# rvp-group/mad-icp

Hardware: NVIDIA H100
Metric: scans/sec (130k-pt scan vs 16-keyframe model) (higher is better)
Workload: dtype f64

## Files before the change

### include/madicp_b200_debug.h

```cpp
#ifndef MADICP_B200_DEBUG_H
#define MADICP_B200_DEBUG_H

#include "madicp_b200.h"

#ifdef __cplusplus
extern "C" {
#endif

int madicp_debug_timing(madicp_ctx_t* ctx, int enable, int64_t* out, int max_rounds);
int madicp_debug_cta_cycles(madicp_ctx_t* ctx, int64_t* out, int cap);
int madicp_debug_cta_stamps(madicp_ctx_t* ctx, int plane, int64_t* out, int cap);
int madicp_set_gn_grid(madicp_ctx_t* ctx, int threads_per_cta, int ctas_per_sm);


int madicp_debug_set_memo(madicp_ctx_t* ctx, int mode);

int64_t madicp_debug_sort_check(int64_t n, uint32_t seed, int64_t distinct, int num_threads);

int64_t madicp_debug_range_mask(const madicp_points_t* desc, uint8_t* keep);

int64_t madicp_debug_correct_points(const madicp_points_t* desc, const madicp_vcorr_t* vcorr, double* out);

int madicp_debug_deskew_plan(const madicp_points_t* desc, const madicp_vcorr_t* vcorr, const double T_prev[12],
                             const double T_now[12], double sensor_hz, int split, int num_threads, int32_t* perm,
                             uint16_t* chunk, double* poses, int* n_poses, int64_t* n_kept);

#ifdef __cplusplus
}
#endif
#endif
```

### mad_icp_b200/_capi.py

```python
import ctypes as C
import os

import numpy as np

_HERE = os.path.dirname(os.path.abspath(__file__))
LIB_PATH = os.path.join(_HERE, "lib", "libmadicp_b200.so")
_lib = None

dp = C.POINTER(C.c_double)
ip = C.POINTER(C.c_int32)
bp = C.POINTER(C.c_uint8)
vp = C.c_void_p


class Points(C.Structure):
    _fields_ = [("data", C.c_void_p), ("n", C.c_int64), ("stride", C.c_int64), ("offset", C.c_int32 * 3),
                ("is_f32", C.c_int32), ("min_range", C.c_double), ("max_range", C.c_double), ("range_mode", C.c_int32),
                ("drop_nan", C.c_int32)]


assert C.sizeof(Points) == 64
pts_p = C.POINTER(Points)


# ... 35 lines not shown
    "madicp_stage_discard": (C.c_int, [vp]),
    "madtree_gpu_upload": (C.c_int, [vp, vp, C.POINTER(vp)]),
    "madtree_gpu_free": (None, [vp]),
    "madtree_gpu_num_nodes": (C.c_int, [vp]),
    "madtree_gpu_num_leaves": (C.c_int, [vp]),
    "madtree_gpu_num_levels": (C.c_int, [vp]),
    "madtree_gpu_download": (C.c_int, [vp, vp, ip]),
    "madtree_gpu_export": (C.c_int, [vp, dp, dp, dp, ip]),
    "madicp_set_moving_tree": (C.c_int, [vp, vp]),
    "madicp_get_moving": (C.c_int, [vp, dp, C.c_int]),
    "madicp_ingest": (C.c_int, [vp, vp, C.c_int64, C.c_int, C.c_int, dp, dp, C.c_double, C.c_int, dp]),
    "madicp_ingest_points": (C.c_int, [vp, pts_p, C.c_int, dp, dp, C.c_double, C.c_int, C.POINTER(C.c_int64), dp]),
    "madicp_stage_points": (C.c_int, [vp, pts_p, C.c_int64]),
    "madtree_gpu_build_batch_points": (C.c_int, [vp, pts_p, C.c_int, C.c_double, C.c_double, C.POINTER(vp)]),
    "madicp_debug_range_mask": (C.c_int64, [pts_p, bp]),
    "madicp_ingest_points_ex": (C.c_int, [vp, pts_p, vc_p, C.c_int, dp, dp, C.c_double, C.c_int, C.POINTER(C.c_int64), dp]),
    "madicp_stage_points_ex": (C.c_int, [vp, pts_p, vc_p, C.c_int64]),
    "madtree_gpu_build_batch_points_ex": (C.c_int, [vp, pts_p, vc_p, C.c_int, C.c_double, C.c_double, C.POINTER(vp)]),
    "madicp_debug_correct_points": (C.c_int64, [pts_p, vc_p, dp]),
    "madicp_plan_points": (C.c_int, [vp, pts_p, vc_p, C.c_int, C.POINTER(vp)]),
    "madicp_ingest_plan": (C.c_int, [vp, vp, C.c_int, dp, dp, C.c_double, C.POINTER(C.c_int64), dp]),
    "madicp_plan_free": (None, [vp]),
    "madicp_debug_deskew_plan": (C.c_int, [pts_p, vc_p, dp, dp, C.c_double, C.c_int, C.c_int, ip,
                                           C.POINTER(C.c_uint16), dp, C.POINTER(C.c_int), C.POINTER(C.c_int64)]),
    "madicp_register_fetch_weight": (C.c_int, [vp, dp, dp, dp, bp, C.POINTER(C.c_int), dp]),
    "madicp_register_partial_async": (C.c_int, [vp, C.c_int, dp]),
    "madicp_calibrate": (C.c_int, [vp, dp]),
    "madicp_drop_keyframe": (C.c_int, [vp, C.c_int]),
    "madicp_num_keyframes": (C.c_int, [vp]),
    "madicp_active_slots": (C.c_int, [vp, ip, C.c_int]),
    "madicp_keyframe_leaves": (C.c_int, [vp, C.c_int]),
    "madicp_set_moving": (C.c_int, [vp, vp, C.c_int]),
    "madicp_search": (C.c_int, [vp, dp, ip]),
    "madicp_linearize": (C.c_int, [vp, dp, dp, dp, bp]),
    "madicp_solve_update": (C.c_int, [vp, dp, dp, dp]),
    "madicp_register": (C.c_int, [vp, C.c_int, dp, dp, dp, bp, C.POINTER(C.c_int)]),
    "madicp_register_async": (C.c_int, [vp, C.c_int, dp]),
    "madicp_register_fetch": (C.c_int, [vp, dp, dp, dp, bp, C.POINTER(C.c_int)]),
    "madicp_register_trace": (C.c_int, [vp, dp, C.c_int]),
    "madicp_register_walked": (C.c_int, [vp, ip, C.c_int]),
    "madicp_register_walk_records": (C.c_int, [vp, C.POINTER(C.c_int64), C.c_int]),
    "madicp_search_cloud": (C.c_int, [vp, C.c_int, dp, C.c_int64, ip, dp, dp, dp]),
    "madicp_deskew": (C.c_int, [dp, C.c_int64, dp, dp, C.c_double, C.c_int]),
    "madicp_debug_sort_check": (C.c_int64, [C.c_int64, C.c_uint32, C.c_int64, C.c_int]),
    "madicp_kernel_launches": (C.c_int64, [vp]),
    "madicp_model_nodes": (C.c_int64, [vp]),
    "madicp_comm_export": (C.c_int, [vp, vp]),
    "madicp_comm_connect": (C.c_int, [vp, C.c_int, C.c_int, vp]),
    "madicp_comm_world": (C.c_int, [vp]),
    "madicp_debug_timing": (C.c_int, [vp, C.c_int, C.POINTER(C.c_int64), C.c_int]),
    "madicp_debug_cta_cycles": (C.c_int, [vp, C.POINTER(C.c_int64), C.c_int]),
    "madicp_set_gn_grid": (C.c_int, [vp, C.c_int, C.c_int]),
    "madicp_debug_set_memo": (C.c_int, [vp, C.c_int]),
    "madicp_debug_cta_stamps": (C.c_int, [vp, C.c_int, C.POINTER(C.c_int64), C.c_int]),
}

REC_DTYPE = np.dtype([("mean", "<f8", 3), ("dir", "<f8", 3), ("bbox0", "<f8"), ("link", "<i4"), ("num_points", "<i4")])
assert REC_DTYPE.itemsize == 64


class MadIcpError(RuntimeError):
    pass


def lib():
    global _lib
    if _lib is None:
        if not os.path.exists(LIB_PATH):
            raise MadIcpError(
                f"{LIB_PATH} is missing: build it with `python -c 'import __graft_entry__ as g; g.build()'` "
                "(make -C mad_icp_b200/csrc).  There is no CPU fallback.")
        L = C.CDLL(LIB_PATH)
        for name, (res, args) in SYMBOLS.items():
            fn = getattr(L, name)
            fn.restype = res
            fn.argtypes = args
        _lib = L
    return _lib


def check(rc, what=""):
    if rc < 0:
        msg = lib().madicp_last_error()
        raise MadIcpError(f"{what} failed ({rc}): {msg.decode() if msg else ''}")
    return rc


def as_d(a):
    return a.ctypes.data_as(dp) if a is not None else None


def as_i(a):
    return a.ctypes.data_as(ip) if a is not None else None


def as_b(a):
    return a.ctypes.data_as(bp) if a is not None else None


def pose12(T):
    T = np.asarray(T, dtype=np.float64)
    if T.shape == (4, 4):
        T = T[:3, :]
    if T.shape != (3, 4):
        raise ValueError("pose must be 4x4 or 3x4")
    return np.ascontiguousarray(T)
# ... 1 lines not shown
```

### mad_icp_b200/csrc/capi.cu

```cuda
#include <cooperative_groups.h>
#include <cuda_runtime.h>

#include <algorithm>
#include <cmath>
#include <cstdio>
#include <cstdlib>
#include <cstring>
#include <new>
#include <stdexcept>
#include <string>
#include <vector>

#include "../../include/madicp_b200_debug.h"
#include "ctx.hpp"
#include "device_kernels.cuh"

namespace madicp {

static thread_local std::string g_error;
void set_error(const std::string& msg) { g_error = msg; }

}

using namespace madicp;
// ... 92 lines not shown
  const int r = int(c->xform_seq % madicp_ctx::kXformRing);
  if (c->xform_seq >= madicp_ctx::kXformRing) CK(cudaEventSynchronize(c->xform_done[r]));
  memcpy(c->h_xform + size_t(r) * 12, X, 12 * sizeof(double));
  CK(cudaMemcpyAsync(c->d_xform + size_t(r) * 12, c->h_xform + size_t(r) * 12, 12 * sizeof(double), cudaMemcpyHostToDevice,
                     c->stream));
  CK(cudaEventRecord(c->xform_done[r], c->stream));
  *X_dev = c->d_xform + size_t(r) * 12;
  c->xform_seq++;
  return MADICP_OK;
}

static int slot_rank(const madicp_ctx* c, int slot) {
  int k = 0;
  for (int s = 0; s < slot; ++s) k += (c->slots[s].n_nodes > 0);
  return k;
}

static int ensure_items(madicp_ctx* c, size_t items) {
  if (items <= c->cap_items) return MADICP_OK;
  CK(cudaStreamSynchronize(c->stream));
  if (c->d_hit) cudaFree(c->d_hit);
  if (c->d_ord) cudaFree(c->d_ord);
  c->d_hit = c->d_ord = nullptr;
  c->cap_items = 0;
  CK(cudaMalloc(&c->d_hit, items * sizeof(int)));
  CK(cudaMalloc(&c->d_ord, items * sizeof(int)));
  c->cap_items = items;
  return MADICP_OK;
}

struct GnShape {
  int threads, ctas;
  const void* fn;
  size_t smem;
};
template <int THREADS, int CTAS>
static GnShape gn_shape() {
  return GnShape{THREADS, CTAS, reinterpret_cast<const void*>(k_gn_loop<THREADS, CTAS>), gn_dynamic_smem<THREADS>()};
}
static const GnShape* gn_shapes(int* n) {
  static const GnShape table[] = {
      gn_shape<1024, 1>(), gn_shape<896, 1>(), gn_shape<768, 1>(), gn_shape<704, 1>(), gn_shape<640, 1>(),
      gn_shape<512, 1>(),  gn_shape<512, 2>(),
      gn_shape<256, 2>(),  gn_shape<256, 3>(), gn_shape<256, 4>(),
  };
  *n = int(sizeof(table) / sizeof(table[0]));
  return table;
}
static int configure_gn(madicp_ctx* c, int threads, int ctas) {
  int n = 0;
  const GnShape* t = gn_shapes(&n);
  for (int i = 0; i < n; ++i)
    if (t[i].threads == threads && t[i].ctas == ctas) {
      CK(cudaFuncSetAttribute(t[i].fn, cudaFuncAttributeMaxDynamicSharedMemorySize, int(t[i].smem + kGnMapMaxBytes)));
      CK(cudaFuncSetAttribute(t[i].fn, cudaFuncAttributePreferredSharedMemoryCarveout,
                              int((t[i].smem * size_t(ctas) + 2048) * 100 / (228 * 1024)) + 1));
      int per_sm = 0;
      CK(cudaOccupancyMaxActiveBlocksPerMultiprocessor(&per_sm, t[i].fn, threads, t[i].smem));
      if (per_sm < ctas) {
        set_error("persistent kernel shape does not fit on an SM");
        return MADICP_ERR_CUDA;
      }
      c->gn_threads = threads;
      c->gn_grid = ctas * c->sm_count;
      c->gn_kernel = t[i].fn;
      c->gn_smem = t[i].smem;
      return MADICP_OK;
    }
  set_error("unsupported persistent-kernel shape (threads per CTA, CTAs per SM)");
  return MADICP_ERR_INVALID;
}

static int pick_shape(madicp_ctx* c, int64_t items) {
  if (!c->gn_auto) return MADICP_OK;
  const double per_sm = double((items + 31) / 32) / double(c->sm_count);
  int best = 1024;
  double best_cost = 1e300;
  for (int i = 0; i < madicp_ctx::kNumAutoShapes; ++i) {
    const int threads = madicp_ctx::kAutoShapes[i];
    const double passes = ceil(per_sm / double(threads / 32));
    const double cost = passes * c->pass_cost[i];
    if (cost < best_cost) {
      best_cost = cost;
      best = threads;
    }
  }
  if (best == c->gn_threads && c->gn_grid == c->sm_count) return MADICP_OK;
  return configure_gn(c, best, 1);
}

static int grid_for(const madicp_ctx* c, int64_t items) {
  int64_t g = (items + kStepBlock - 1) / kStepBlock;
  const int64_t cap = int64_t(c->sm_count) * 8;
  if (g > cap) g = cap;
  if (g < 1) g = 1;
  return int(g);
}

extern "C" {

const char* madicp_last_error(void) { return g_error.c_str(); }
int madicp_abi_version(void) { return 3; }

int madicp_create(madicp_ctx_t** out, int device, int max_keyframes) {
  if (!out || max_keyframes < 1 || max_keyframes > kMaxSlots) {
    set_error("madicp_create: bad arguments (1 <= max_keyframes <= 64)");
    return MADICP_ERR_INVALID;
  }
  MADICP_TRY
  int n_dev = 0;
  cudaError_t e = cudaGetDeviceCount(&n_dev);
  if (e != cudaSuccess || n_dev <= 0 || device < 0 || device >= n_dev) {
    set_error(std::string("madicp_create: no usable CUDA device (") +
              (e != cudaSuccess ? cudaGetErrorString(e) : "device index out of range") +
              "); this library has no CPU fallback");
    return MADICP_ERR_CUDA;
  }
  CK(cudaSetDevice(device));
  cudaDeviceProp prop;
  CK(cudaGetDeviceProperties(&prop, device));
  if (prop.major != 9 || prop.minor != 0) {
    set_error("madicp_create: device is not sm_90 (H100); kernels are built for sm_90a only");
    return MADICP_ERR_CUDA;
  }
  madicp_ctx* c = new madicp_ctx;
  c->device = device;
  c->max_keyframes = max_keyframes;
  c->sm_count = prop.multiProcessorCount;
  c->slots.resize(max_keyframes);
  {
    int lo_pri = 0, hi_pri = 0;
    CK(cudaDeviceGetStreamPriorityRange(&lo_pri, &hi_pri));
    CK(cudaStreamCreateWithPriority(&c->own_stream, cudaStreamNonBlocking, hi_pri));
  }
  c->stream = c->own_stream;
  CK(cudaMalloc(&c->d_state, sizeof(GnState)));
  CK(cudaMemset(c->d_state, 0, sizeof(GnState)));
  CK(cudaMalloc(&c->d_X, sizeof(double) * 64));
  CK(cudaMalloc(&c->d_comm, sizeof(CommBlock)));
  CK(cudaMemset(c->d_comm, 0, sizeof(CommBlock)));
  CK(cudaEventCreateWithFlags(&c->tree_free_ev, cudaEventDisableTiming));
  CK(cudaMalloc(&c->d_pool_lvl, size_t(max_keyframes) * (kMaxLevels + 1) * sizeof(int)));
  CK(cudaMalloc(&c->d_xform, size_t(madicp_ctx::kXformRing) * 12 * sizeof(double)));
  CK(cudaMallocHost(&c->h_xform, size_t(madicp_ctx::kXformRing) * 12 * sizeof(double)));
  CK(cudaMallocHost(&c->h_lvl, size_t(madicp_ctx::kXformRing) * (kMaxLevels + 1) * sizeof(int)));
  for (int i = 0; i < madicp_ctx::kXformRing; ++i) CK(cudaEventCreateWithFlags(&c->xform_done[i], cudaEventDisableTiming));
  CK(cudaMallocHost(&c->h_pinned, sizeof(double) * 64));
  CK(cudaMallocHost(&c->h_state, sizeof(GnState)));
  CK(cudaMallocHost(&c->h_matched, kMatchedCap));
  if (const char* e = getenv("MADICP_NO_MEMO")) c->memo_mode = (atoi(e) == 0) ? 2 : 0;
  int threads = 1024, ctas = 1;
  if (const char* e = getenv("MADICP_GN_SHAPE"))
    if (sscanf(e, "%d,%d", &threads, &ctas) == 2) c->gn_auto = false;
  int rc = configure_gn(c, threads, ctas);
  if (rc) return rc;
  c->cap_partial = size_t(c->sm_count) * 8 * kAcc;
  CK(cudaMalloc(&c->d_partial, c->cap_partial * sizeof(double)));
  CK(cudaMalloc(&c->d_tiles, c->cap_partial * sizeof(LLCell)));
  CK(cudaMemset(c->d_tiles, 0, c->cap_partial * sizeof(LLCell)));
  c->peer_comm[0] = c->d_comm;
  *out = c;
  return MADICP_OK;
  MADICP_CATCH("madicp_create")
}

void madicp_destroy(madicp_ctx_t* c) {
  if (!c) return;
  cudaSetDevice(c->device);
  cudaStreamSynchronize(c->stream);
  for (int r = 0; r < c->world; ++r)
    if (c->world > 1 && r != c->rank && c->peer_comm[r]) cudaIpcCloseMemHandle(c->peer_comm[r]);
  madicp_gpu_build_release(c);
  for (madtree_gpu* t : c->tree_cache) delete t;
  for (void* slab : c->tree_slabs) cudaFree(slab);
  cudaFree(c->d_pool_recs);
  cudaFree(c->d_pool_child0);
  cudaFree(c->d_pool_rec_of);
  cudaFree(c->d_pool_lvl);
  cudaFree(c->d_quad);
  cudaFree(c->d_pool_ww);
  cudaFree(c->d_xform);
  cudaFree(c->d_dbg_cta);
  cudaFree(c->d_moving);
  cudaFree(c->d_mov4);
  cudaFree(c->d_step_matched);
  cudaFree(c->d_hit);
  cudaFree(c->d_ord);
  cudaFree(c->d_cloud_q);
  cudaFree(c->d_cloud_o);
  cudaFree(c->d_partial);
  cudaFree(c->d_tiles);
  cudaFree(c->d_memo_leaf);
  cudaFree(c->d_memo_margin);
  cudaFree(c->d_memo_ckpt);
  cudaFree(c->d_memo_ckpt_up);
  cudaFree(c->d_state);
  cudaFree(c->d_X);
  cudaFree(c->d_comm);
  cudaFree(c->d_dbg);
  cudaFreeHost(c->h_xform);
  cudaFreeHost(c->h_lvl);
  cudaFreeHost(c->h_pinned);
  cudaFreeHost(c->h_state);
// ... 467 lines not shown
  CK(cudaMemcpyAsync(c->h_state, c->d_state, offsetof(GnState, X_trace), cudaMemcpyDeviceToHost, c->stream));
  if (matched) CK(cudaMemcpyAsync(c->h_matched, c->d_step_matched, size_t(c->L), cudaMemcpyDeviceToHost, c->stream));
  CK(cudaStreamSynchronize(c->stream));
  memcpy(H, c->h_state->H, sizeof(double) * 36);
  memcpy(b, c->h_state->b, sizeof(double) * 6);
  if (matched) memcpy(matched, c->h_matched, size_t(c->L));
  return MADICP_OK;
}

int madicp_solve_update(madicp_ctx_t* c, const double H[36], const double b[6], double X[12]) {
  if (!c || !H || !b || !X) return MADICP_ERR_INVALID;
  CK(cudaSetDevice(c->device));
  memcpy(c->h_pinned, X, 12 * sizeof(double));
  memcpy(c->h_pinned + 12, H, 36 * sizeof(double));
  memcpy(c->h_pinned + 48, b, 6 * sizeof(double));
  CK(cudaMemcpyAsync(c->d_X, c->h_pinned, 54 * sizeof(double), cudaMemcpyHostToDevice, c->stream));
  k_solve<<<1, 32, 0, c->stream>>>(c->d_X + 12, c->d_X + 48, c->d_X);
  c->launches++;
  CK(cudaGetLastError());
  CK(cudaMemcpyAsync(c->h_pinned, c->d_X, 12 * sizeof(double), cudaMemcpyDeviceToHost, c->stream));
  CK(cudaStreamSynchronize(c->stream));
  memcpy(X, c->h_pinned, 12 * sizeof(double));
  return MADICP_OK;
}

static int register_enqueue(madicp_ctx* c, int iters, const double X0[12], int clear_from) {
  int rc = check_ready(c, "madicp_register");
  if (rc) return rc;
  if (!X0 || iters < 1 || iters > MADICP_MAX_ITERS) {
    set_error("madicp_register: bad arguments (1 <= iters <= 64 per launch)");
    return MADICP_ERR_INVALID;
  }
  CK(cudaSetDevice(c->device));
  rc = prepare_moving(c);
  if (rc) return rc;
  rc = pick_shape(c, int64_t(madicp_num_keyframes(c)) * c->L);
  if (rc) return rc;
  GnArgs A;
  A.model = make_view(c);
  A.P = c->P;
  A.peers.rank = c->rank;
  A.peers.world = c->world;
  A.peers.epoch_base = c->epoch;
  const int mb = int(c->call_seq & 1u);
  for (int r = 0; r < kMaxPeers; ++r) {
    A.peers.box[r] = (r < c->world) ? &c->peer_comm[r]->box : nullptr;
    A.peer_matched[r] = (r < c->world) ? c->peer_comm[r]->matched[mb] : nullptr;
  }
  A.moving = c->d_mov4;
  A.L = c->L;
  A.iters = iters;
  A.clear_from = clear_from;
  A.matched = c->d_comm->matched[mb];
  size_t map_bytes = 0;
  {
    const size_t per_cta = size_t(madicp_num_keyframes(c)) * (size_t(c->L) / size_t(c->gn_grid) + 8) * 4 + 128;
    auto bucket = [](size_t bytes) {
      const size_t kb[] = {8, 16, 32, 64, 100, 132, 164, 196, 228};
      for (size_t b : kb)
        if (bytes + 1024 <= b * 1024) return b;
      return size_t(1 << 20);
    };
    const size_t ctas = size_t(c->gn_grid / c->sm_count);
    if (per_cta <= kGnMapMaxBytes && c->L < (1 << 26) && bucket((c->gn_smem + per_cta) * ctas) == bucket(c->gn_smem * ctas))
      map_bytes = per_cta;
  }
  A.map_in_smem = map_bytes ? 1 : 0;
  {
    const size_t stride = ((size_t(c->max_keyframes) * (c->cap_moving / size_t(c->gn_grid) + 8)) + 31) & ~size_t(31);
    const size_t need = stride * size_t(c->gn_grid);
    if (need > c->cap_memo) {
      CK(cudaStreamSynchronize(c->stream));
      cudaFree(c->d_memo_leaf);
      cudaFree(c->d_memo_margin);
      cudaFree(c->d_memo_ckpt);
      cudaFree(c->d_memo_ckpt_up);
      c->d_memo_leaf = nullptr;
      c->d_memo_margin = nullptr;
      c->d_memo_ckpt = nullptr;
      c->d_memo_ckpt_up = nullptr;
      c->cap_memo = 0;
      const size_t cap = need + need / 4;
      CK(cudaMalloc(&c->d_memo_leaf, cap * sizeof(int)));
      CK(cudaMalloc(&c->d_memo_margin, cap * sizeof(float)));
      CK(cudaMalloc(&c->d_memo_ckpt, cap * sizeof(unsigned)));
      CK(cudaMalloc(&c->d_memo_ckpt_up, cap * sizeof(float)));
      c->cap_memo = cap;
    }
    A.memo_leaf = c->d_memo_leaf;
    A.memo_margin = c->d_memo_margin;
    A.memo_ckpt = c->d_memo_ckpt;
    A.memo_ckpt_up = c->d_memo_ckpt_up;
    A.item_stride = int(stride);
    A.memo_mode = c->memo_mode;
    A.walk_buf = mb;
  }
  A.st = c->d_state;
  A.dbg = c->d_dbg;
  A.dbg_cta = c->d_dbg ? c->d_dbg_cta : nullptr;
  c->epoch += uint32_t(iters);
  A.pose_epoch = c->pose_epoch;
  c->pose_epoch += uint32_t(iters);
  memcpy(A.X0, X0, 12 * sizeof(double));
  A.tiles = c->d_tiles;
  A.zero_next = c->d_comm->matched[mb ^ 1];
  A.zero_bytes = int((std::min(kMatchedCap, c->cap_moving) + 15) & ~size_t(15));
  void* args[] = {&A};
  CK(cudaLaunchCooperativeKernel(c->gn_kernel, dim3(c->gn_grid), dim3(c->gn_threads), args, c->gn_smem + map_bytes, c->stream));
  c->launches++;
  c->last_iters = iters;
  c->call_seq++;
  return MADICP_OK;
}

int madicp_register_async(madicp_ctx_t* c, int iters, const double X0[12]) {
  return register_enqueue(c, iters, X0, iters - 1);
}
int madicp_register_partial_async(madicp_ctx_t* c, int iters, const double X0[12]) {
  return register_enqueue(c, iters, X0, 0);
}

int madicp_register_fetch_weight(madicp_ctx_t* c, double X[12], double H[36], double b[6], uint8_t* matched, int* n_matched,
                                 double* weight) {
  if (!c || c->last_iters < 1) {
    set_error("madicp_register_fetch: nothing was enqueued");
    return MADICP_ERR_STATE;
  }
  CK(cudaSetDevice(c->device));
  CK(cudaMemcpyAsync(c->h_state, c->d_state, offsetof(GnState, X_trace), cudaMemcpyDeviceToHost, c->stream));
  if (matched)
    CK(cudaMemcpyAsync(c->h_matched, c->d_comm->matched[(c->call_seq - 1u) & 1u], size_t(c->L), cudaMemcpyDeviceToHost,
                       c->stream));
  CK(cudaStreamSynchronize(c->stream));
  if (c->h_state->error) {
    set_error("madicp_register: a peer GPU never delivered its H/b tile (rank down, or no matching registration enqueued there)");
    CK(cudaMemsetAsync(&c->d_state->error, 0, sizeof(int), c->stream));
    return MADICP_ERR_COMM;
  }
  if (X) memcpy(X, c->h_state->X_out, 12 * sizeof(double));
  if (H) memcpy(H, c->h_state->H, 36 * sizeof(double));
  if (b) memcpy(b, c->h_state->b, 6 * sizeof(double));
  if (matched) memcpy(matched, c->h_matched, size_t(c->L));
  if (n_matched) *n_matched = c->h_state->n_matched;
  if (weight) *weight = c->h_state->weight;
  return MADICP_OK;
}
int madicp_register_fetch(madicp_ctx_t* c, double X[12], double H[36], double b[6], uint8_t* matched, int* n_matched) {
  return madicp_register_fetch_weight(c, X, H, b, matched, n_matched, nullptr);
}

int madicp_register(madicp_ctx_t* c, int iters, double X[12], double H[36], double b[6], uint8_t* matched,
                    int* n_matched) {
  if (!c || !X || iters < 0) {
    set_error("madicp_register: bad arguments");
    return MADICP_ERR_INVALID;
  }
  if (iters == 0) {
    if (H) memset(H, 0, 36 * sizeof(double));
    if (b) memset(b, 0, 6 * sizeof(double));
    if (matched && c->L > 0) memset(matched, 0, size_t(c->L));
    if (n_matched) *n_matched = 0;
// ... 172 lines not shown
}

int madicp_debug_timing(madicp_ctx_t* c, int enable, int64_t* out, int max_rounds) {
  if (!c) return MADICP_ERR_INVALID;
  CK(cudaSetDevice(c->device));
  CK(cudaStreamSynchronize(c->stream));
  int rows = 0;
  if (out && c->d_dbg) {
    rows = std::min(max_rounds, c->last_iters);
    CK(cudaMemcpy(out, c->d_dbg, size_t(rows) * 8 * sizeof(long long), cudaMemcpyDeviceToHost));
  }
  if (enable && !c->d_dbg) {
    CK(cudaMalloc(&c->d_dbg, MADICP_MAX_ITERS * 8 * sizeof(long long)));
    CK(cudaMemset(c->d_dbg, 0, MADICP_MAX_ITERS * 8 * sizeof(long long)));
    CK(cudaMalloc(&c->d_dbg_cta, size_t(MADICP_MAX_ITERS) * c->sm_count * 8 * 4 * sizeof(long long)));
    CK(cudaMemset(c->d_dbg_cta, 0, size_t(MADICP_MAX_ITERS) * c->sm_count * 8 * 4 * sizeof(long long)));
  } else if (!enable && c->d_dbg) {
    cudaFree(c->d_dbg);
    cudaFree(c->d_dbg_cta);
    c->d_dbg = nullptr;
    c->d_dbg_cta = nullptr;
  }
  return rows;
}

int madicp_debug_cta_cycles(madicp_ctx_t* c, int64_t* out, int cap) {
  if (!c || !out || !c->d_dbg_cta) return MADICP_ERR_INVALID;
  CK(cudaSetDevice(c->device));
  CK(cudaStreamSynchronize(c->stream));
  const int n = std::min(cap, c->last_iters * c->gn_grid);
  CK(cudaMemcpy(out, c->d_dbg_cta, size_t(n) * sizeof(long long), cudaMemcpyDeviceToHost));
  return c->gn_grid;
}

int madicp_debug_cta_stamps(madicp_ctx_t* c, int plane, int64_t* out, int cap) {
  if (!c || !out || !c->d_dbg_cta || plane < 0 || plane > 4) return MADICP_ERR_INVALID;
  CK(cudaSetDevice(c->device));
  CK(cudaStreamSynchronize(c->stream));
  const int n = std::min(cap, c->last_iters * c->gn_grid);
  CK(cudaMemcpy(out, c->d_dbg_cta + size_t(plane) * MADICP_MAX_ITERS * c->gn_grid, size_t(n) * sizeof(long long),
                cudaMemcpyDeviceToHost));
  return c->gn_grid;
}

int madicp_debug_set_memo(madicp_ctx_t* c, int mode) {
  if (!c || mode < 0 || mode > 2) {
    set_error("madicp_debug_set_memo: mode must be 0 (off), 1 (leaf memo) or 2 (leaf memo + resume)");
    return MADICP_ERR_INVALID;
  }
  c->memo_mode = mode;
  return MADICP_OK;
}

int madicp_set_gn_grid(madicp_ctx_t* c, int threads_per_cta, int ctas_per_sm) {
  if (!c || ctas_per_sm < 1) return MADICP_ERR_INVALID;
  CK(cudaSetDevice(c->device));
  if (threads_per_cta == 0) {
    c->gn_auto = true;
    return 0;
  }
  int rc = configure_gn(c, threads_per_cta, ctas_per_sm);
  if (rc) return rc;
  c->gn_auto = false;
  return c->gn_grid / c->sm_count;
}

}
```

### mad_icp_b200/csrc/ctx.hpp

```cpp
#pragma once
#include <cuda_runtime.h>

#include <atomic>
#include <mutex>
#include <new>
#include <stdexcept>
#include <string>
#include <vector>

#include "kernels.cuh"

namespace madicp {
void set_error(const std::string& msg);

constexpr int kMaxLevels = 4096;
struct Slot {
  int n_nodes = 0, n_leaves = 0, n_levels = 0;
};
constexpr size_t kMatchedCap = size_t(1) << 20;

struct CommBlock {
  Mailbox box;
  unsigned char matched[2][kMatchedCap];
};
// ... 15 lines not shown
  uint64_t build_seq = 0;
};

struct madicp_ctx {
  int device = 0;
  int max_keyframes = 0;
  cudaStream_t own_stream = nullptr, stream = nullptr;
  int sm_count = 0;
  std::vector<madicp::Slot> slots;
  size_t pool_cap = 0;
  madtree_rec_t* d_pool_recs = nullptr;
  int* d_pool_child0 = nullptr;
  int* d_pool_rec_of = nullptr;
  int* d_pool_lvl = nullptr;
  size_t quad_cap = 0;
  madicp::QuadRec* d_quad = nullptr;
  double* d_pool_ww = nullptr;
  static constexpr int kXformRing = 64;
  double* d_xform = nullptr;
  double* h_xform = nullptr;
  int* h_lvl = nullptr;
  cudaEvent_t xform_done[kXformRing] = {};
  uint32_t xform_seq = 0;
  std::vector<madtree_gpu*> tree_cache;
  std::vector<void*> tree_slabs;
  cudaEvent_t tree_free_ev = nullptr;
  std::mutex tree_mu;
  void* build_state = nullptr;
  void* plan_state = nullptr;
  long long* d_dbg_cta = nullptr;
  madicp::IcpParams P{0.2, 0.31622776601683794, 0.02};
  double* d_moving = nullptr;
  madicp::Moving4* d_mov4 = nullptr;
  bool mov4_stale = true;
  unsigned char* d_step_matched = nullptr;
  int L = 0;
  size_t cap_moving = 0;
  uint32_t call_seq = 0;
  int* d_hit = nullptr;
  int* d_ord = nullptr;
  size_t cap_items = 0;
  double* d_cloud_q = nullptr;
  int* d_cloud_o = nullptr;
  size_t cap_cloud = 0;
  double* d_partial = nullptr;
  madicp::LLCell* d_tiles = nullptr;
  size_t cap_partial = 0;
  int* d_memo_leaf = nullptr;
  float* d_memo_margin = nullptr;
  unsigned* d_memo_ckpt = nullptr;
  float* d_memo_ckpt_up = nullptr;
  size_t cap_memo = 0;
  int memo_mode = 2;
  madicp::GnState* d_state = nullptr;
  double* d_X = nullptr;
  madicp::CommBlock* d_comm = nullptr;
  double* h_pinned = nullptr;
  madicp::GnState* h_state = nullptr;
  unsigned char* h_matched = nullptr;
  int gn_grid = 0;
  bool gn_auto = true;
  int gn_threads = 1024;
  const void* gn_kernel = nullptr;
  size_t gn_smem = 0;
  static constexpr int kNumAutoShapes = 6;
  static constexpr int kAutoShapes[kNumAutoShapes] = {768, 1024, 896, 704, 640, 512};
  double pass_cost[kNumAutoShapes] = {5570.0, 8260.0, 7480.0, 5650.0, 5325.0, 4650.0};
  bool calibrated = false;
  int last_iters = 0;
  long long* d_dbg = nullptr;
  std::atomic<int64_t> launches{0};
  int rank = 0, world = 1;
  madicp::CommBlock* peer_comm[madicp::kMaxPeers] = {};
  uint32_t epoch = 0;
  uint32_t pose_epoch = 1;
};

#define CK(call)                                                                                   \
  do {                                                                                             \
    cudaError_t e_ = (call);                                                                       \
    if (e_ != cudaSuccess) {                                                                       \
      madicp::set_error(std::string(#call) + ": " + cudaGetErrorString(e_));                       \
      return MADICP_ERR_CUDA;                                                                      \
    }                                                                                              \
  } while (0)

#define MADICP_TRY try {
#define MADICP_CATCH(who)                                          \
  }                                                                \
  catch (const std::bad_alloc&) {                                  \
    madicp::set_error(std::string(who) + ": out of host memory");  \
    return MADICP_ERR_NOMEM;                                       \
  }                                                                \
  catch (const std::exception& e_) {                               \
    madicp::set_error(std::string(who) + ": " + e_.what());        \
    return MADICP_ERR_INVALID;                                     \
  }

int madicp_tree_alloc(madicp_ctx* c, size_t cap_nodes, madtree_gpu** out);
void madicp_gpu_build_release(madicp_ctx* c);
```

### mad_icp_b200/csrc/device_kernels.cuh

```cuda
#pragma once
#include "kernels.cuh"

namespace madicp {


__device__ __forceinline__ int depth_of(const int* __restrict__ lvl, int n_levels, int i) {
  int lo = 0, hi = n_levels;
  while (hi - lo > 1) {
    const int mid = (lo + hi) >> 1;
    if (__ldg(lvl + mid) <= i) lo = mid; else hi = mid;
  }
  return lo;
}

__global__ void __launch_bounds__(kStepBlock)
k_slot_ingest(const madtree_rec_t* src, madtree_rec_t* dst, int n, const double* __restrict__ Xp,
              const int* __restrict__ lvl, int n_levels, int* __restrict__ flag) {
  const int i = blockIdx.x * kStepBlock + threadIdx.x;
  if (i >= n) return;
  Rec r = load_rec_plain(src + i);
  const int npts = src[i].num_points;
  int f = 0;
  if (r.link >= 0 && (depth_of(lvl, n_levels, i) & 1) == 0)
    f = (src[r.link].link >= 0 || src[r.link + 1].link >= 0) ? 1 : 0;
// ... 229 lines not shown
k_search_cloud(const __grid_constant__ ModelView model, int root, const double* __restrict__ q, int64_t n,
               int* __restrict__ ordinals, double* __restrict__ points, double* __restrict__ normals,
               double* __restrict__ dists) {
  for (int64_t i = int64_t(blockIdx.x) * kStepBlock + threadIdx.x; i < n; i += int64_t(gridDim.x) * kStepBlock) {
    const double qx = q[3 * i], qy = q[3 * i + 1], qz = q[3 * i + 2];
    double ww;
    const Rec f = load_rec(model.recs + descend(model, root, qx, qy, qz, ww));
    if (ordinals) ordinals[i] = -1 - f.link;
    if (points) {
      points[3 * i] = f.mx; points[3 * i + 1] = f.my; points[3 * i + 2] = f.mz;
    }
    if (normals) {
      normals[3 * i] = f.dx; normals[3 * i + 1] = f.dy; normals[3 * i + 2] = f.dz;
    }
    if (dists) dists[i] = norm3(qx - f.mx, qy - f.my, qz - f.mz);
  }
}


template <int THREADS>
__device__ __forceinline__ void peer_allreduce(const PeerView& pv, uint32_t epoch, double* s_tot,
                                               double (*s_peer)[kAcc], int* error) {
  const int slot = int(epoch & 1u);
  for (int idx = threadIdx.x; idx < pv.world * kAcc; idx += THREADS) {
    const int r = idx / kAcc, i = idx - r * kAcc;
    const double v = s_tot[i];
    const uint32_t lo = uint32_t(__double2loint(v)), hi = uint32_t(__double2hiint(v));
    LLCell* dst = &pv.box[r]->cell[slot][pv.rank][i];
    asm volatile("st.volatile.global.v4.u32 [%0], {%1,%2,%3,%4};" ::"l"(dst), "r"(lo), "r"(epoch), "r"(hi), "r"(epoch)
                 : "memory");
  }
  for (int idx = threadIdx.x; idx < pv.world * kAcc; idx += THREADS) {
    const int r = idx / kAcc, i = idx - r * kAcc;
    const LLCell* src = &pv.box[pv.rank]->cell[slot][r][i];
    uint32_t lo, f0, hi, f1, spins = 0;
    do {
      asm volatile("ld.volatile.global.v4.u32 {%0,%1,%2,%3}, [%4];" : "=r"(lo), "=r"(f0), "=r"(hi), "=r"(f1) : "l"(src)
                   : "memory");
      if (++spins == (1u << 26)) {
        *error = 1;
        break;
      }
    } while (f0 != epoch || f1 != epoch);
    s_peer[r][i] = __hiloint2double(int(hi), int(lo));
  }
  __syncthreads();
  if (threadIdx.x < kAcc) {
    double s = s_peer[0][threadIdx.x];
    for (int r = 1; r < pv.world; ++r) s += s_peer[r][threadIdx.x];
    s_tot[threadIdx.x] = s;
  }
  __syncthreads();
}

struct GnArgs {
  ModelView model;
  IcpParams P;
  PeerView peers;
  const Moving4* moving;
  int L;
  int iters;
  int clear_from;
  unsigned char* matched;
  unsigned char* peer_matched[kMaxPeers];
  LLCell* tiles;
  double X0[12];
  unsigned char* zero_next;
  int zero_bytes;
  GnState* st;
  int map_in_smem;
  uint32_t pose_epoch;
  int* memo_leaf;
  float* memo_margin;
  unsigned* memo_ckpt;
  float* memo_ckpt_up;
  int item_stride;
  int walk_buf;
  int memo_mode;
  long long* dbg;
  long long* dbg_cta;
};
#ifndef MADICP_CKPT_TAU_SCALE
#define MADICP_CKPT_TAU_SCALE 1.0
#endif
__device__ __forceinline__ float ckpt_tau(int it, double moved, double ball) {
  return __double2float_ru(MADICP_CKPT_TAU_SCALE * (it == 0 ? ball : moved));
}

__device__ __forceinline__ long long global_ns() {
  long long t;
  asm volatile("mov.u64 %0, %%globaltimer;" : "=l"(t));
  return t;
}

template <int THREADS, int CTAS>
__global__ void __launch_bounds__(THREADS, CTAS)
k_gn_loop(const __grid_constant__ GnArgs A) {
  constexpr int WARPS = THREADS / 32;
  extern __shared__ __align__(16) double s_dyn[];
  double* s_stage_all = s_dyn;
  double(*s_red)[64] = reinterpret_cast<double(*)[64]>(s_dyn);
  double(*s_peer)[kAcc] = reinterpret_cast<double(*)[kAcc]>(s_dyn + WARPS * 64);
  static_assert(WARPS * 64 + kMaxPeers * kAcc <= WARPS * kStageTile, "scratch must fit in the staging tiles");
  __shared__ double s_tot[kAcc];
  __shared__ double s_b[6];
  __shared__ double s_X[12], s_Xp[12];
  __shared__ int s_qn, s_rn;
  __shared__ int s_count[WARPS];
  GnState* st = A.st;
  const unsigned L = unsigned(A.L);
  const unsigned total = unsigned(A.model.K) * L;
  const bool multi = A.peers.world > 1;
  const unsigned lane = threadIdx.x & 31;
  const unsigned warp = threadIdx.x >> 5;
  double* stage = s_stage_all + warp * kStageTile;
  constexpr unsigned kPieces = 4;
  unsigned p_lo[kPieces], p_n[kPieces];
  unsigned n_b = 0;
#pragma unroll
  const unsigned G = gridDim.x;
  const unsigned light = (G >= 8u) ? 3u : 0u;
  const uint64_t W8 = 8ull * G - light;
  for (unsigned p = 0; p < kPieces; ++p) {
    const unsigned s = (p & 1u) ? (G - 1u - blockIdx.x) : blockIdx.x;
    auto cum8 = [&](unsigned pos) -> uint64_t {
      if (p & 1u) return (pos >= G) ? W8 : 8ull * pos;
      return pos ? 8ull * pos - light : 0ull;
    };
    const uint64_t p0 = (uint64_t(L) * p) / kPieces, p1 = (uint64_t(L) * (p + 1)) / kPieces;
    const unsigned lo = unsigned(p0 + ((p1 - p0) * cum8(s)) / W8);
    const unsigned hi = unsigned(p0 + ((p1 - p0) * cum8(s + 1u)) / W8);
    p_lo[p] = lo;
    p_n[p] = hi - lo;
    n_b += p_n[p];
  }
  const unsigned t_total = unsigned(A.model.K) * n_b;
  (void) total;
  auto item_of = [&](unsigned t0, unsigned& k, unsigned& q) {
    k = t0 / n_b;
    q = t0 - k * n_b + lane;
    while (q >= n_b) {
      q -= n_b;
      ++k;
    }
    const unsigned j = q;
    q = p_lo[kPieces - 1] + (j - (n_b - p_n[kPieces - 1]));
    unsigned acc = 0;
#pragma unroll
    for (unsigned p = 0; p + 1 < kPieces; ++p) {
      if (j >= acc && j < acc + p_n[p]) q = p_lo[p] + (j - acc);
      acc += p_n[p];
    }
  };
  unsigned* s_map = A.map_in_smem ? reinterpret_cast<unsigned*>(s_dyn + WARPS * kStageTile) : nullptr;
  if (s_map) {
    for (unsigned t0 = warp * 32; t0 < t_total; t0 += THREADS) {
      unsigned k, q;
      item_of(t0, k, q);
      s_map[t0 + lane] = (k << 26) | q;
    }
    __syncwarp();
  }

  for (int i = (blockIdx.x * THREADS + threadIdx.x) * 16; i < A.zero_bytes; i += gridDim.x * THREADS * 16)
    *reinterpret_cast<uint4*>(A.zero_next + i) = make_uint4(0, 0, 0, 0);
  if (blockIdx.x == 0 && threadIdx.x < MADICP_MAX_ITERS) {
    st->walked[A.walk_buf ^ 1][threadIdx.x] = 0;
    st->walk_recs[A.walk_buf ^ 1][threadIdx.x] = 0;
  }
  int* const memo_leaf = A.memo_leaf + size_t(blockIdx.x) * A.item_stride;
  float* const memo_margin = A.memo_margin + size_t(blockIdx.x) * A.item_stride;
  unsigned* const memo_ckpt = A.memo_ckpt + size_t(blockIdx.x) * A.item_stride;
  float* const memo_ckpt_up = A.memo_ckpt_up + size_t(blockIdx.x) * A.item_stride;
  auto item_at = [&](unsigned t0, unsigned& k, unsigned& q) {
    if (s_map) {
      const unsigned pk = s_map[t0 + lane];
      k = pk >> 26;
      q = pk & 0x3ffffffu;
    } else {
      item_of(t0, k, q);
    }
  };

  for (int it = 0; it < A.iters; ++it) {
    if (threadIdx.x < 12) {
      double x;
      if (it == 0) {
        x = A.X0[threadIdx.x];
      } else {
        const uint32_t ep = A.pose_epoch + uint32_t(it);
        uint32_t lo, hi, f0, f1;
        do {
          ll_load(&st->X_ll[threadIdx.x], lo, f0, hi, f1);
        } while (f0 != ep || f1 != ep);
        x = __hiloint2double(int(hi), int(lo));
      }
      s_Xp[threadIdx.x] = s_X[threadIdx.x];
      s_X[threadIdx.x] = x;
      if (it == 0 && blockIdx.x == 0) st->X_trace[threadIdx.x] = x;
    }
    if (threadIdx.x == 32) s_qn = 0;
    if (threadIdx.x == 33) s_rn = 0;
    __syncthreads();
    const bool last_round = (it == A.iters - 1);
    double c0 = 0.0, c1 = 0.0;
    long long t_begin = 0;
    if (A.dbg && threadIdx.x == 0) t_begin = clock64();
    const size_t dbg_plane = size_t(MADICP_MAX_ITERS) * gridDim.x, dbg_at = size_t(it) * gridDim.x + blockIdx.x;
    if (A.dbg_cta && threadIdx.x == 0) A.dbg_cta[dbg_plane + dbg_at] = global_ns();

    int n_walked = 0, n_recs = 0;
    for (unsigned t0 = warp * 32; t0 < t_total; t0 += THREADS) {
      unsigned k, q;
      item_at(t0, k, q);
      double v[kStage];
#pragma unroll
      for (int i = 0; i < kStage; ++i) v[i] = 0.0;
      const unsigned t = t0 + lane;
      if (t < t_total) {
        const Moving4 m = load_moving(A.moving + q);
        double mx, my, mz;
        iso_apply(s_X, m.px, m.py, m.pz, mx, my, mz);
        int leaf = -1;
        Rec f;
        double ww = 0.0;
        unsigned start = 0;
        float prefix = __int_as_float(0x7f800000);
        double moved = 0.0;
        if (it > 0 && A.memo_mode) {
          const float have = memo_margin[t];
          const int last = memo_leaf[t];
          unsigned ck = 0;
          float ck_up = 0.0f;
          if (A.memo_mode == 2) {
            ck = memo_ckpt[t];
            ck_up = memo_ckpt_up[t];
          }
          f = load_rec(A.model.recs + last);
          ww = __ldg(A.model.ww + last);
          double bx, by, bz;
          iso_apply(s_Xp, m.px, m.py, m.pz, bx, by, bz);
          const double dx = mx - bx, dy = my - by, dz = mz - bz;
          moved = 1.0001 * sqrt(dx * dx + dy * dy + dz * dz) + 1e-9 + 1e-12 * (fabs(mx) + fabs(my) + fabs(mz));
          const double left = double(have) - moved;
          if (left > 0.0) {
            memo_margin[t] = __double2float_rd(left);
            leaf = last;
          } else if (ck != 0) {
            const double ck_left = __dsub_rd(__dadd_rd(double(have), double(ck_up)), moved);
            if (ck_left > 0.0) {
              start = ck;
              prefix = __double2float_rd(ck_left);
            }
          }
        }
        if (leaf < 0) {
          double ww_walk;
          const float tau = ckpt_tau(it, moved, m.ball);
          float margin = prefix, ck_margin = 0.0f;
          unsigned ckpt = start;
          leaf = A.memo_mode ? descend_t<true>(A.model, int(k), mx, my, mz, ww_walk, margin, ckpt, ck_margin, tau, n_recs)
                             : descend_t<false>(A.model, int(k), mx, my, mz, ww_walk, margin, ckpt, ck_margin, tau, n_recs);
          if (A.memo_mode) {
            memo_leaf[t] = leaf;
            memo_margin[t] = margin;
          }
          if (A.memo_mode == 2) {
            memo_ckpt[t] = ckpt;
            memo_ckpt_up[t] = __fsub_rd(ck_margin, margin);
          }
          ++n_walked;
          ww = __ldg(A.model.ww + leaf);
          f = load_rec(A.model.recs + leaf);
        }
        if (linearize_one(s_X, A.P.rho_ker_sqrt, m, mx, my, mz, f, ww, v) && it >= A.clear_from) {
          if (multi) {
            for (int r = 0; r < A.peers.world; ++r) A.peer_matched[r][q] = 1;
          } else {
            A.matched[q] = 1;
          }
        }
      }
      warp_accumulate(stage, v, c0, c1);
    }
    n_walked = __reduce_add_sync(0xffffffffu, n_walked);
    n_recs = __reduce_add_sync(0xffffffffu, n_recs);
    if (lane == 0 && n_walked) {
      atomicAdd(&s_qn, n_walked);
      atomicAdd(&s_rn, n_recs);
    }
    if (A.dbg && threadIdx.x == 0 && blockIdx.x == 0) A.dbg[it * 8 + 0] = clock64() - t_begin;
    if (A.dbg_cta) {
      __syncthreads();
      if (threadIdx.x == 0) {
        A.dbg_cta[dbg_at] = clock64() - t_begin;
        A.dbg_cta[2 * dbg_plane + dbg_at] = global_ns();
// ... 85 lines not shown
```

### mad_icp_b200/engine.py

```python
import ctypes as C
import math

import numpy as np

from . import _capi as capi
from ._capi import MadIcpError, as_b, as_d, as_i, check, pose12
from .records import VERTICAL_ANGLE_OFFSET, describe, vcorr


class FlatTree:

    def __init__(self, points, b_max=0.2, b_min=0.1, num_threads=1):
        pts = np.ascontiguousarray(points, dtype=np.float64)
        if pts.ndim != 2 or pts.shape[1] != 3:
            raise ValueError("points must be N x 3")
        h = C.c_void_p()
        check(capi.lib().madtree_build(as_d(pts), pts.shape[0], b_max, b_min, num_threads, C.byref(h)), "madtree_build")
        self._h = h
        self.b_max, self.b_min = b_max, b_min

    def __del__(self):
        h = getattr(self, "_h", None)
        if h:
            self._h = None
# ... 342 lines not shown
        n, w = C.c_int(0), C.c_double(0)
        check(capi.lib().madicp_register_fetch_weight(self._h, as_d(X), as_d(H), as_d(b), as_b(m), C.byref(n), C.byref(w)),
              "madicp_register_fetch")
        return dict(X=X, H=H, b=b, matched=m, n_matched=n.value, weight=w.value)

    def register_trace(self):
        buf = np.empty((65, 3, 4))
        rows = check(capi.lib().madicp_register_trace(self._h, as_d(buf), 65), "madicp_register_trace")
        return buf[:rows].copy()

    def register_walked(self):
        buf = np.zeros(64, np.int32)
        rows = check(capi.lib().madicp_register_walked(self._h, as_i(buf), 64), "madicp_register_walked")
        return buf[:rows].copy()

    def register_walk_records(self):
        buf = np.zeros(64, np.int64)
        rows = check(capi.lib().madicp_register_walk_records(self._h, buf.ctypes.data_as(C.POINTER(C.c_int64)), 64),
                     "madicp_register_walk_records")
        return buf[:rows].copy()

    def search_cloud(self, slot, queries, want=("ordinals", "points", "normals", "dists")):
        q = np.ascontiguousarray(queries, dtype=np.float64).reshape(-1, 3)
        n = q.shape[0]
        o = np.empty(n, np.int32) if "ordinals" in want else None
        p = np.empty((n, 3)) if "points" in want else None
        nr = np.empty((n, 3)) if "normals" in want else None
        d = np.empty(n) if "dists" in want else None
        check(capi.lib().madicp_search_cloud(self._h, slot, as_d(q), n, as_i(o), as_d(p), as_d(nr), as_d(d)),
              "madicp_search_cloud")
        return dict(ordinals=o, points=p, normals=nr, dists=d)

    def debug_timing(self, enable=True, fetch=True):
        buf = np.zeros((64, 8), np.int64)
        rows = check(capi.lib().madicp_debug_timing(self._h, int(enable), buf.ctypes.data_as(C.POINTER(C.c_int64))
                                                    if fetch else None, 64))
        return buf[:rows]

    def debug_cta_cycles(self, rounds):
        buf = np.zeros(rounds * 2048, np.int64)
        grid = check(capi.lib().madicp_debug_cta_cycles(self._h, buf.ctypes.data_as(C.POINTER(C.c_int64)), buf.size))
        return buf[:rounds * grid].reshape(rounds, grid)

    def debug_cta_stamps(self, plane, rounds):
        buf = np.zeros(rounds * 2048, np.int64)
        grid = check(capi.lib().madicp_debug_cta_stamps(self._h, plane, buf.ctypes.data_as(C.POINTER(C.c_int64)), buf.size))
        return buf[:rounds * grid].reshape(rounds, grid)

    def set_memo(self, mode=True):
        if isinstance(mode, bool):
            mode = 2 if mode else 0
        check(capi.lib().madicp_debug_set_memo(self._h, int(mode)), "madicp_debug_set_memo")

    def set_gn_grid(self, threads_per_cta=1024, ctas_per_sm=1):
        return check(capi.lib().madicp_set_gn_grid(self._h, threads_per_cta, ctas_per_sm))

    def comm_export(self):
        buf = (C.c_char * 64)()
        check(capi.lib().madicp_comm_export(self._h, buf), "madicp_comm_export")
        return bytes(buf)

    def comm_connect(self, rank, world, handles):
        blob = b"".join(handles)
        assert len(blob) == 64 * world
        check(capi.lib().madicp_comm_connect(self._h, rank, world, blob), "madicp_comm_connect")

    @property
    def world(self):
        return capi.lib().madicp_comm_world(self._h)


__all__ = ["FlatTree", "DeviceTree", "Registrar", "MadIcpError"]
```

Measured before the change: 4965.

## Cache per-leaf moving points and transformed positions in a shared-memory query table

Each CTA now builds a shared-memory table of its moving leaves (original point, ball, leaf index). Once per GN iteration it computes the transformed position and memo move distance for each leaf, so the K keyframe work items for the same leaf reuse them instead of reloading from global memory and recomputing the transform. The table is enabled only when it fits in 16KB and does not change the shared-memory occupancy bucket, and it takes priority over the item map for shared space. The cost is an extra per-iteration pass plus a __syncthreads, more shared memory, and possibly losing the smem item map.

```diff
diff --git a/include/madicp_b200_debug.h b/include/madicp_b200_debug.h
--- a/include/madicp_b200_debug.h
+++ b/include/madicp_b200_debug.h
@@ -15,6 +15,9 @@
 
 int madicp_debug_set_memo(madicp_ctx_t* ctx, int mode);
 
+int madicp_debug_set_query_table(madicp_ctx_t* ctx, int enable);
+int madicp_debug_query_table_leaves(madicp_ctx_t* ctx);
+
 int64_t madicp_debug_sort_check(int64_t n, uint32_t seed, int64_t distinct, int num_threads);
 
 int64_t madicp_debug_range_mask(const madicp_points_t* desc, uint8_t* keep);
diff --git a/mad_icp_b200/_capi.py b/mad_icp_b200/_capi.py
--- a/mad_icp_b200/_capi.py
+++ b/mad_icp_b200/_capi.py
@@ -111,6 +111,8 @@
     "madicp_debug_cta_cycles": (C.c_int, [vp, C.POINTER(C.c_int64), C.c_int]),
     "madicp_set_gn_grid": (C.c_int, [vp, C.c_int, C.c_int]),
     "madicp_debug_set_memo": (C.c_int, [vp, C.c_int]),
+    "madicp_debug_set_query_table": (C.c_int, [vp, C.c_int]),
+    "madicp_debug_query_table_leaves": (C.c_int, [vp]),
     "madicp_debug_cta_stamps": (C.c_int, [vp, C.c_int, C.POINTER(C.c_int64), C.c_int]),
 }
 
diff --git a/mad_icp_b200/csrc/capi.cu b/mad_icp_b200/csrc/capi.cu
--- a/mad_icp_b200/csrc/capi.cu
+++ b/mad_icp_b200/csrc/capi.cu
@@ -168,7 +168,7 @@
   const GnShape* t = gn_shapes(&n);
   for (int i = 0; i < n; ++i)
     if (t[i].threads == threads && t[i].ctas == ctas) {
-      CK(cudaFuncSetAttribute(t[i].fn, cudaFuncAttributeMaxDynamicSharedMemorySize, int(t[i].smem + kGnMapMaxBytes)));
+      CK(cudaFuncSetAttribute(t[i].fn, cudaFuncAttributeMaxDynamicSharedMemorySize, int(t[i].smem + kGnQtabMaxBytes + kGnMapMaxBytes)));
       CK(cudaFuncSetAttribute(t[i].fn, cudaFuncAttributePreferredSharedMemoryCarveout,
                               int((t[i].smem * size_t(ctas) + 2048) * 100 / (228 * 1024)) + 1));
       int per_sm = 0;
@@ -265,6 +265,7 @@
   CK(cudaMallocHost(&c->h_state, sizeof(GnState)));
   CK(cudaMallocHost(&c->h_matched, kMatchedCap));
   if (const char* e = getenv("MADICP_NO_MEMO")) c->memo_mode = (atoi(e) == 0) ? 2 : 0;
+  if (const char* e = getenv("MADICP_NO_QTAB")) c->qtab_enabled = atoi(e) == 0;
   int threads = 1024, ctas = 1;
   if (const char* e = getenv("MADICP_GN_SHAPE"))
     if (sscanf(e, "%d,%d", &threads, &ctas) == 2) c->gn_auto = false;
@@ -838,9 +839,9 @@
   A.iters = iters;
   A.clear_from = clear_from;
   A.matched = c->d_comm->matched[mb];
-  size_t map_bytes = 0;
+  size_t qtab_bytes = 0, map_bytes = 0;
+  const size_t cta_leaves = size_t(c->L) / size_t(c->gn_grid) + 8;
   {
-    const size_t per_cta = size_t(madicp_num_keyframes(c)) * (size_t(c->L) / size_t(c->gn_grid) + 8) * 4 + 128;
     auto bucket = [](size_t bytes) {
       const size_t kb[] = {8, 16, 32, 64, 100, 132, 164, 196, 228};
       for (size_t b : kb)
@@ -848,9 +849,15 @@
       return size_t(1 << 20);
     };
     const size_t ctas = size_t(c->gn_grid / c->sm_count);
-    if (per_cta <= kGnMapMaxBytes && c->L < (1 << 26) && bucket((c->gn_smem + per_cta) * ctas) == bucket(c->gn_smem * ctas))
+    const size_t own = bucket(c->gn_smem * ctas);
+    const size_t qtab = gn_qtab_doubles(unsigned(std::min(cta_leaves, size_t(1) << 20))) * sizeof(double);
+    if (c->qtab_enabled && qtab <= kGnQtabMaxBytes && bucket((c->gn_smem + qtab) * ctas) == own) qtab_bytes = qtab;
+    const size_t per_cta = size_t(madicp_num_keyframes(c)) * cta_leaves * 4 + 128;
+    if (per_cta <= kGnMapMaxBytes && c->L < (1 << 26) && bucket((c->gn_smem + qtab_bytes + per_cta) * ctas) == own)
       map_bytes = per_cta;
   }
+  A.qtab_cap = qtab_bytes ? int(cta_leaves) : 0;
+  c->last_qtab_cap = A.qtab_cap;
   A.map_in_smem = map_bytes ? 1 : 0;
   {
     const size_t stride = ((size_t(c->max_keyframes) * (c->cap_moving / size_t(c->gn_grid) + 8)) + 31) & ~size_t(31);
@@ -892,7 +899,8 @@
   A.zero_next = c->d_comm->matched[mb ^ 1];
   A.zero_bytes = int((std::min(kMatchedCap, c->cap_moving) + 15) & ~size_t(15));
   void* args[] = {&A};
-  CK(cudaLaunchCooperativeKernel(c->gn_kernel, dim3(c->gn_grid), dim3(c->gn_threads), args, c->gn_smem + map_bytes, c->stream));
+  CK(cudaLaunchCooperativeKernel(c->gn_kernel, dim3(c->gn_grid), dim3(c->gn_threads), args, c->gn_smem + qtab_bytes + map_bytes,
+                                c->stream));
   c->launches++;
   c->last_iters = iters;
   c->call_seq++;
@@ -1171,6 +1179,14 @@
   return MADICP_OK;
 }
 
+int madicp_debug_set_query_table(madicp_ctx_t* c, int enable) {
+  if (!c) return MADICP_ERR_INVALID;
+  c->qtab_enabled = enable != 0;
+  return MADICP_OK;
+}
+
+int madicp_debug_query_table_leaves(madicp_ctx_t* c) { return c ? c->last_qtab_cap : MADICP_ERR_INVALID; }
+
 int madicp_set_gn_grid(madicp_ctx_t* c, int threads_per_cta, int ctas_per_sm) {
   if (!c || ctas_per_sm < 1) return MADICP_ERR_INVALID;
   CK(cudaSetDevice(c->device));
diff --git a/mad_icp_b200/csrc/ctx.hpp b/mad_icp_b200/csrc/ctx.hpp
--- a/mad_icp_b200/csrc/ctx.hpp
+++ b/mad_icp_b200/csrc/ctx.hpp
@@ -91,6 +91,8 @@
   float* d_memo_ckpt_up = nullptr;
   size_t cap_memo = 0;
   int memo_mode = 2;
+  bool qtab_enabled = true;
+  int last_qtab_cap = 0;
   madicp::GnState* d_state = nullptr;
   double* d_X = nullptr;
   madicp::CommBlock* d_comm = nullptr;
diff --git a/mad_icp_b200/csrc/device_kernels.cuh b/mad_icp_b200/csrc/device_kernels.cuh
--- a/mad_icp_b200/csrc/device_kernels.cuh
+++ b/mad_icp_b200/csrc/device_kernels.cuh
@@ -305,6 +305,9 @@
   }
   __syncthreads();
 }
+
+__host__ __device__ constexpr size_t gn_qtab_doubles(unsigned cap) { return size_t(cap) * 8 + (size_t(cap) + 1) / 2; }
+constexpr size_t kGnQtabMaxBytes = 16 * 1024;
 
 struct GnArgs {
   ModelView model;
@@ -322,6 +325,7 @@
   int zero_bytes;
   GnState* st;
   int map_in_smem;
+  int qtab_cap;
   uint32_t pose_epoch;
   int* memo_leaf;
   float* memo_margin;
@@ -338,6 +342,14 @@
 #endif
 __device__ __forceinline__ float ckpt_tau(int it, double moved, double ball) {
   return __double2float_ru(MADICP_CKPT_TAU_SCALE * (it == 0 ? ball : moved));
+}
+
+__device__ __forceinline__ double charged_move(const double* Xp, double px, double py, double pz, double mx, double my,
+                                               double mz) {
+  double bx, by, bz;
+  iso_apply(Xp, px, py, pz, bx, by, bz);
+  const double dx = mx - bx, dy = my - by, dz = mz - bz;
+  return 1.0001 * sqrt(dx * dx + dy * dy + dz * dz) + 1e-9 + 1e-12 * (fabs(mx) + fabs(my) + fabs(mz));
 }
 
 __device__ __forceinline__ long long global_ns() {
@@ -389,28 +401,47 @@
   }
   const unsigned t_total = unsigned(A.model.K) * n_b;
   (void) total;
-  auto item_of = [&](unsigned t0, unsigned& k, unsigned& q) {
-    k = t0 / n_b;
-    q = t0 - k * n_b + lane;
-    while (q >= n_b) {
-      q -= n_b;
-      ++k;
-    }
-    const unsigned j = q;
-    q = p_lo[kPieces - 1] + (j - (n_b - p_n[kPieces - 1]));
+  auto leaf_at = [&](unsigned j) {
+    unsigned q = p_lo[kPieces - 1] + (j - (n_b - p_n[kPieces - 1]));
     unsigned acc = 0;
 #pragma unroll
     for (unsigned p = 0; p + 1 < kPieces; ++p) {
       if (j >= acc && j < acc + p_n[p]) q = p_lo[p] + (j - acc);
       acc += p_n[p];
     }
+    return q;
   };
-  unsigned* s_map = A.map_in_smem ? reinterpret_cast<unsigned*>(s_dyn + WARPS * kStageTile) : nullptr;
+  constexpr unsigned kQx = 0, kQy = 1, kQz = 2, kQmoved = 3, kQpx = 4, kQpy = 5, kQpz = 6, kQball = 7, kQfields = 8;
+  const unsigned pitch = unsigned(A.qtab_cap);
+  double* const s_qtab = s_dyn + WARPS * kStageTile;
+  unsigned* const s_qleaf = reinterpret_cast<unsigned*>(s_qtab + kQfields * pitch);
+  const bool qt = pitch != 0 && n_b <= pitch;
+  if (qt) {
+    for (unsigned j = threadIdx.x; j < n_b; j += THREADS) {
+      const unsigned q = leaf_at(j);
+      const Moving4 m = load_moving(A.moving + q);
+      s_qtab[kQpx * pitch + j] = m.px;
+      s_qtab[kQpy * pitch + j] = m.py;
+      s_qtab[kQpz * pitch + j] = m.pz;
+      s_qtab[kQball * pitch + j] = m.ball;
+      s_qleaf[j] = q;
+    }
+  }
+  auto item_of = [&](unsigned t0, unsigned& k, unsigned& x) {
+    k = t0 / n_b;
+    unsigned j = t0 - k * n_b + lane;
+    while (j >= n_b) {
+      j -= n_b;
+      ++k;
+    }
+    x = qt ? j : leaf_at(j);
+  };
+  unsigned* s_map = A.map_in_smem ? reinterpret_cast<unsigned*>(s_qtab + (pitch ? gn_qtab_doubles(pitch) : 0)) : nullptr;
   if (s_map) {
     for (unsigned t0 = warp * 32; t0 < t_total; t0 += THREADS) {
-      unsigned k, q;
-      item_of(t0, k, q);
-      s_map[t0 + lane] = (k << 26) | q;
+      unsigned k, x;
+      item_of(t0, k, x);
+      s_map[t0 + lane] = (k << 26) | x;
     }
     __syncwarp();
   }
@@ -425,13 +456,13 @@
   float* const memo_margin = A.memo_margin + size_t(blockIdx.x) * A.item_stride;
   unsigned* const memo_ckpt = A.memo_ckpt + size_t(blockIdx.x) * A.item_stride;
   float* const memo_ckpt_up = A.memo_ckpt_up + size_t(blockIdx.x) * A.item_stride;
-  auto item_at = [&](unsigned t0, unsigned& k, unsigned& q) {
+  auto item_at = [&](unsigned t0, unsigned& k, unsigned& x) {
     if (s_map) {
       const unsigned pk = s_map[t0 + lane];
       k = pk >> 26;
-      q = pk & 0x3ffffffu;
+      x = pk & 0x3ffffffu;
     } else {
-      item_of(t0, k, q);
+      item_of(t0, k, x);
     }
   };
 
@@ -455,6 +486,18 @@
     if (threadIdx.x == 32) s_qn = 0;
     if (threadIdx.x == 33) s_rn = 0;
     __syncthreads();
+    if (qt) {
+      for (unsigned j = threadIdx.x; j < n_b; j += THREADS) {
+        const double px = s_qtab[kQpx * pitch + j], py = s_qtab[kQpy * pitch + j], pz = s_qtab[kQpz * pitch + j];
+        double mx, my, mz;
+        iso_apply(s_X, px, py, pz, mx, my, mz);
+        s_qtab[kQx * pitch + j] = mx;
+        s_qtab[kQy * pitch + j] = my;
+        s_qtab[kQz * pitch + j] = mz;
+        if (it > 0 && A.memo_mode) s_qtab[kQmoved * pitch + j] = charged_move(s_Xp, px, py, pz, mx, my, mz);
+      }
+      __syncthreads();
+    }
     const bool last_round = (it == A.iters - 1);
     double c0 = 0.0, c1 = 0.0;
     long long t_begin = 0;
@@ -464,16 +507,30 @@
 
     int n_walked = 0, n_recs = 0;
     for (unsigned t0 = warp * 32; t0 < t_total; t0 += THREADS) {
-      unsigned k, q;
-      item_at(t0, k, q);
+      unsigned k, x;
+      item_at(t0, k, x);
       double v[kStage];
 #pragma unroll
       for (int i = 0; i < kStage; ++i) v[i] = 0.0;
       const unsigned t = t0 + lane;
       if (t < t_total) {
-        const Moving4 m = load_moving(A.moving + q);
+        unsigned q;
+        Moving4 m;
         double mx, my, mz;
-        iso_apply(s_X, m.px, m.py, m.pz, mx, my, mz);
+        if (qt) {
+          q = s_qleaf[x];
+          m.px = s_qtab[kQpx * pitch + x];
+          m.py = s_qtab[kQpy * pitch + x];
+          m.pz = s_qtab[kQpz * pitch + x];
+          m.ball = s_qtab[kQball * pitch + x];
+          mx = s_qtab[kQx * pitch + x];
+          my = s_qtab[kQy * pitch + x];
+          mz = s_qtab[kQz * pitch + x];
+        } else {
+          q = x;
+          m = load_moving(A.moving + q);
+          iso_apply(s_X, m.px, m.py, m.pz, mx, my, mz);
+        }
         int leaf = -1;
         Rec f;
         double ww = 0.0;
@@ -491,10 +548,7 @@
           }
           f = load_rec(A.model.recs + last);
           ww = __ldg(A.model.ww + last);
-          double bx, by, bz;
-          iso_apply(s_Xp, m.px, m.py, m.pz, bx, by, bz);
-          const double dx = mx - bx, dy = my - by, dz = mz - bz;
-          moved = 1.0001 * sqrt(dx * dx + dy * dy + dz * dz) + 1e-9 + 1e-12 * (fabs(mx) + fabs(my) + fabs(mz));
+          moved = qt ? s_qtab[kQmoved * pitch + x] : charged_move(s_Xp, m.px, m.py, m.pz, mx, my, mz);
           const double left = double(have) - moved;
           if (left > 0.0) {
             memo_margin[t] = __double2float_rd(left);
diff --git a/mad_icp_b200/engine.py b/mad_icp_b200/engine.py
--- a/mad_icp_b200/engine.py
+++ b/mad_icp_b200/engine.py
@@ -418,6 +418,12 @@
             mode = 2 if mode else 0
         check(capi.lib().madicp_debug_set_memo(self._h, int(mode)), "madicp_debug_set_memo")
 
+    def set_query_table(self, enable=True):
+        check(capi.lib().madicp_debug_set_query_table(self._h, int(bool(enable))), "madicp_debug_set_query_table")
+
+    def query_table_leaves(self):
+        return check(capi.lib().madicp_debug_query_table_leaves(self._h), "madicp_debug_query_table_leaves")
+
     def set_gn_grid(self, threads_per_cta=1024, ctas_per_sm=1):
         return check(capi.lib().madicp_set_gn_grid(self._h, threads_per_cta, ctas_per_sm))
 
```

After: 5020, median of 6. 1.01x the previous value.
